# arclabs561/innr

Measured on NVIDIA B200. Metric: batch_knn_cosine_top10_queries_per_s, higher is better.
Workload: dtype f32

## Files before the change

innr_b200/csrc/scan_f32.cu:

```cuda
#include <algorithm>
#include <cmath>
#include <type_traits>

#include "common.cuh"
#include "kernels.cuh"
#include "pdx.cuh"

namespace innr {

namespace {

constexpr int SCAN_THREADS = 256;
constexpr int VPT = 4;
constexpr int TILE = SCAN_THREADS * VPT;
constexpr float NORM_EPS = 1e-9f;

struct PdxArgs {
  PdxView v;
  unsigned long long ld;
  unsigned n, d, ld4;
  unsigned n_tiles;
  unsigned index_base;
  const float* queries;
  int nq_valid;
  int k;
  uint64_t* partials;
  uint64_t* out_keys;
  uint64_t* group_partials;
  unsigned* tickets;
  float* scores_out;
  const float* norms_in;
  const uint32_t* mask;
  const uint32_t* perm;
  float threshold;
  float one;
  const unsigned* run_flag;
};

template <int MODE>
__device__ __forceinline__ void accumulate(float q, float v, float& acc) {
  if (MODE == PDX_L2 || MODE == PDX_L2_PRUNE || MODE == PDX_L2_PERM) {
    float diff = __fsub_rn(q, v);
    acc = __fadd_rn(acc, __fmul_rn(diff, diff));
  } else {
    acc = __fadd_rn(acc, __fmul_rn(q, v));
  }
}

template <int MODE>
__device__ __forceinline__ void accumulate2(uint64_t q2, uint64_t v2, uint64_t& acc2, uint64_t one2) {
  if (MODE == PDX_L2 || MODE == PDX_L2_PRUNE || MODE == PDX_L2_PERM) {
    const uint64_t diff = sub2_rn(q2, v2);
    acc2 = add2_unfusable(mul2_rn(diff, diff), acc2, one2);
  } else {
    acc2 = add2_unfusable(mul2_rn(q2, v2), acc2, one2);
  }
}

template <int MODE, int QB, int R, bool KNN, bool MASKED = false, int UX = 0>
// ... 943 lines not shown
  ++*launches;
  return cudaGetLastError();
}

cudaError_t launch_adaptive_epoch(const PdxView& v, const float* dev_query, size_t d0, size_t d1, float* dev_dist,
                                  const uint32_t* dev_mask_in, uint32_t* dev_mask_out, const float* dev_thr, uint32_t* dev_ev,
                                  unsigned* dev_pruned, int no_prune, cudaStream_t s, LaunchCounter* launches) {
  AdaptArgs a{};
  a.v = v;
  a.ld = v.ld;
  a.ld4 = (unsigned)std::min<size_t>(v.ld, (v.n + 3) / 4 * 4);
  a.query = dev_query;
  a.d0 = (unsigned)d0;
  a.d1 = (unsigned)d1;
  a.dist = dev_dist;
  a.mask_in = dev_mask_in;
  a.mask_out = dev_mask_out;
  a.thr = dev_thr;
  a.ev = dev_ev;
  a.pruned = dev_pruned;
  a.no_prune = no_prune;
  const unsigned span = (a.ld4 + 31u) / 32u * 32u;
  const unsigned grid = (span / VPT + SCAN_THREADS - 1) / SCAN_THREADS;
  adaptive_epoch_kernel<<<grid, SCAN_THREADS, (d1 - d0) * sizeof(float), s>>>(a);
  ++*launches;
  return cudaGetLastError();
}

cudaError_t launch_adaptive_event_keys(const uint32_t* dev_before, const uint32_t* dev_after, const uint32_t* dev_ev, size_t n,
                                       uint64_t* dev_keys, cudaStream_t s, LaunchCounter* launches) {
  adaptive_event_keys_kernel<<<(unsigned)((n + SCAN_THREADS - 1) / SCAN_THREADS), SCAN_THREADS, 0, s>>>(dev_before, dev_after,
                                                                                                     dev_ev, (unsigned)n, dev_keys);
  ++*launches;
  return cudaGetLastError();
}

cudaError_t launch_adaptive_revive(const uint64_t* dev_keys, size_t m, uint32_t* dev_mask, cudaStream_t s,
                                   LaunchCounter* launches) {
  if (m == 0) return cudaSuccess;
  adaptive_revive_kernel<<<(unsigned)((m + 255) / 256), 256, 0, s>>>(dev_keys, (unsigned)m, dev_mask);
  ++*launches;
  return cudaGetLastError();
}

cudaError_t launch_topk_from_distances(const float* dev_dist, size_t n, size_t k, uint64_t* dev_keys,
                                       Workspace& ws, cudaStream_t s, LaunchCounter* launches) {
  return launch_topk_from_scores(dev_dist, 0, n, 0, k, dev_keys, ws, s, launches, nullptr, nullptr, 1, 1);
}

namespace {

constexpr int SC_VPT = 16;
constexpr int SC_TILE = SCAN_THREADS * SC_VPT;
constexpr int SC_U = 8;
constexpr int RS_WARPS = 4;

struct ScreenArgs {
  PdxSketch sk;
  unsigned long long ld;
  unsigned n, d, ld16, n_tiles, index_base;
  int k;
  const float* query;
  const float* norms;
  float gamma, eta, nu;
  uint64_t* partials;
  uint64_t* group_partials;
  unsigned* tickets;
  uint64_t* tkeys;
  float* opt;
  float* pess;
  unsigned* ctl;
};

struct alignas(16) ScreenQuery {
  float qn_ref, qn_up;
  float qq_lo, qq_hi;
  float q128;
  float e1;
  float gq;
  float unscale;
  unsigned wmax[SCAN_THREADS / 32];
};

template <int MODE>
__device__ __forceinline__ void screen_bounds(float acc, float s, float r, float nv, const ScreenQuery& c,
                                              const ScreenArgs& a, float& lower, float& upper) {
  const float g = a.gamma;
  const float v_up = __fmul_ru(__fadd_ru(__fmul_ru(nv, 1.0f + 0x1p-23f), a.nu), __fadd_ru(1.0f, g));
  if (!(__fmul_ru(c.qn_up, v_up) <= 0x1p100f)) {
    lower = -INFINITY;
    upper = INFINITY;
    return;
  }
  const float m_lo = __fsub_rd(__fsub_rd(__fmul_rd(acc, c.unscale), c.q128), c.e1);
  const float m_hi = __fadd_ru(__fsub_ru(__fmul_ru(acc, c.unscale), c.q128), c.e1);
  const float qr = __fmul_ru(c.qn_up, r);
  const float x_lo = __fsub_rd(__fmul_rd(s, m_lo), qr);
  const float x_hi = __fadd_ru(__fmul_ru(s, m_hi), qr);
  if (MODE == PDX_L2) {
    const float n_lo = __fmul_rd(nv, 1.0f - 0x1p-23f);
    const float vv_lo = fmaxf(0.0f, __fmul_rd(__fsub_rd(__fmul_rd(n_lo, n_lo), a.eta), __fsub_rd(1.0f, g)));
    const float l_lo = fmaxf(0.0f, __fadd_rd(__fsub_rd(c.qq_lo, 2.0f * x_hi), vv_lo));
    const float l_hi = __fadd_ru(__fsub_ru(c.qq_hi, 2.0f * x_lo), __fmul_ru(v_up, v_up));
    lower = fmaxf(0.0f, __fsub_rd(__fmul_rd(l_lo, __fsub_rd(1.0f, g)), a.eta));
    upper = __fadd_ru(__fmul_ru(l_hi, __fadd_ru(1.0f, g)), a.eta);
    if (!(upper <= 3.0e38f)) { lower = -INFINITY; upper = INFINITY; }
    return;
  }
  const float e = __fmaf_ru(c.gq, v_up, a.eta);
  lower = __fsub_rd(x_lo, e);
  upper = __fadd_ru(x_hi, e);
  if (MODE == PDX_COSINE_FUSED) {
    if (!(nv > NORM_EPS)) {
      lower = upper = 0.0f;
      return;
    }
    const float p = __fmul_rn(c.qn_ref, nv);
    lower = __fdiv_rd(lower, p);
    upper = __fdiv_ru(upper, p);
  }
}

template <int MODE, int R>
__global__ void __launch_bounds__(SCAN_THREADS) pdx_screen_kernel(const ScreenArgs a) {
  extern __shared__ __align__(16) unsigned char smem_raw[];
  const unsigned d_pad = (a.d + 31u) / 32u * 32u;
  float* sq = reinterpret_cast<float*>(smem_raw);
  float* sqs = sq + d_pad;
  ScreenQuery* sc = reinterpret_cast<ScreenQuery*>(sqs + d_pad);
  uint64_t* smem_keys = reinterpret_cast<uint64_t*>(sc + 1);
  const int lane = threadIdx.x & 31;
  unsigned mb = 0;
  for (unsigned dd = threadIdx.x; dd < d_pad; dd += blockDim.x) {
    const float x = dd < a.d ? a.query[dd] : 0.0f;
    sq[dd] = x;
    mb = max(mb, __float_as_uint(x) & 0x7FFFFFFFu);
  }
  mb = __reduce_max_sync(FULL_MASK, mb);
  if (lane == 0) sc->wmax[threadIdx.x >> 5] = mb;
  __syncthreads();
#pragma unroll
  for (int w = 0; w < SCAN_THREADS / 32; ++w) mb = max(mb, sc->wmax[w]);
  if (!(mb >= 0x0D800000u && mb <= 0x71800000u)) {
    if (threadIdx.x == 0) a.ctl[1] = 1u;
    return;
  }
  const int p = 253 - (int)(mb >> 23);
  const float f1 = __uint_as_float((unsigned)(p / 2 + 127) << 23), f2 = __uint_as_float((unsigned)(p - p / 2 + 127) << 23);
  for (unsigned dd = threadIdx.x; dd < d_pad; dd += blockDim.x) sqs[dd] = __fmul_rn(__fmul_rn(sq[dd], f1), f2);
  __syncthreads();
  if (threadIdx.x == SCAN_THREADS - 1) {
    float ss = 0.0f, su = 0.0f, sl = 0.0f, qs = 0.0f, sa = 0.0f;
    for (unsigned dd = 0; dd < a.d; ++dd) {
      const float x = sq[dd];
      ss = __fadd_rn(ss, __fmul_rn(x, x));
      su = __fmaf_ru(x, x, su);
      sl = __fmaf_rd(x, x, sl);
      qs = __fadd_rn(qs, x);
      sa = __fadd_ru(sa, fabsf(x));
    }
    const float us = __uint_as_float((unsigned)(276 - p) << 23);
    sc->qn_ref = __fsqrt_rn(ss);
    sc->qn_up = __fsqrt_ru(su);
    sc->qq_lo = sl;
    sc->qq_hi = su;
    sc->q128 = 128.0f * qs;
    sc->e1 = __fadd_ru(__fmul_ru(a.gamma, __fmul_ru(383.0f, sa)), __fmul_ru(__uint_as_float(a.d), us));
    sc->gq = __fmul_ru(a.gamma, sc->qn_up);
    sc->unscale = us;
  }
  bool qn_visible = false;
  WarpList<R> lists[1];
  lists[0].init();
  uint64_t thr = KEY_SENTINEL;

  for (unsigned tile = blockIdx.x; tile < a.n_tiles; tile += gridDim.x) {
    const unsigned i0 = tile * SC_TILE + threadIdx.x * SC_VPT;
    const bool active = i0 < a.ld16;
    uint64_t acc[SC_VPT / 2];
#pragma unroll
    for (int j = 0; j < SC_VPT / 2; ++j) acc[j] = 0;
    auto step = [&](const uint4& w, float q) {
      const uint64_t q2 = pack2(q, q);
      const unsigned x[4] = {w.x, w.y, w.z, w.w};
#pragma unroll
      for (int t = 0; t < 4; ++t) {
        const float b0 = __uint_as_float(__byte_perm(x[t], 0u, 0x4440u)), b1 = __uint_as_float(__byte_perm(x[t], 0u, 0x4441u));
        const float b2 = __uint_as_float(__byte_perm(x[t], 0u, 0x4442u)), b3 = __uint_as_float(__byte_perm(x[t], 0u, 0x4443u));
        acc[2 * t] = fma2_rn(q2, pack2(b0, b1), acc[2 * t]);
        acc[2 * t + 1] = fma2_rn(q2, pack2(b2, b3), acc[2 * t + 1]);
      }
    };
    if (active) {
      const uint8_t* p = a.sk.codes + pdx_sketch_off(a.ld, 0, i0);
      const size_t next = pdx_sketch_off(a.ld, 1, 0);
      unsigned dd = 0;
      for (; dd + SC_U <= a.d; dd += SC_U) {
        uint4 w[SC_U];
#pragma unroll
        for (int u = 0; u < SC_U; ++u) w[u] = ldg_stream_u4(reinterpret_cast<const uint4*>(p + u * next));
        p += SC_U * next;
#pragma unroll
        for (int u = 0; u < SC_U; ++u) step(w[u], sqs[dd + u]);
      }
      for (; dd < a.d; ++dd, p += next) step(ldg_stream_u4(reinterpret_cast<const uint4*>(p)), sqs[dd]);
    }
    if (!qn_visible) {
      __syncthreads();
      qn_visible = true;
      const float qr = sc->qn_ref, qu = sc->qn_up;
      if (!(qu <= 0x1p100f) || (MODE == PDX_COSINE_FUSED && !(qr >= NORM_EPS))) {
        if (threadIdx.x == 0) a.ctl[1] = 1u;
        return;
      }
    }
#pragma unroll
    for (int h = 0; h < SC_VPT / 4; ++h) {
      const unsigned ih = i0 + 4 * h;
      float lo[4] = {0.0f, 0.0f, 0.0f, 0.0f}, up[4] = {0.0f, 0.0f, 0.0f, 0.0f};
      if (active) {
        const float4 s4 = *reinterpret_cast<const float4*>(a.sk.scale + ih);
        const float4 r4 = *reinterpret_cast<const float4*>(a.sk.resid + ih);
        const float4 n4 = *reinterpret_cast<const float4*>(a.norms + ih);
        const float s[4] = {s4.x, s4.y, s4.z, s4.w}, r[4] = {r4.x, r4.y, r4.z, r4.w}, nv[4] = {n4.x, n4.y, n4.z, n4.w};
        float x[4];
        unpack2(acc[2 * h], x[0], x[1]);
        unpack2(acc[2 * h + 1], x[2], x[3]);
#pragma unroll
        for (int j = 0; j < 4; ++j) screen_bounds<MODE>(x[j], s[j], r[j], nv[j], *sc, a, lo[j], up[j]);
        const float* ob = (MODE == PDX_L2) ? lo : up;
        *reinterpret_cast<float4*>(a.opt + ih) = make_float4(ob[0], ob[1], ob[2], ob[3]);
        if (a.pess) {
          const float* pb = (MODE == PDX_L2) ? up : lo;
          for (int j = 0; j < 4; ++j) a.pess[ih + j] = pb[j];
        }
      }
#pragma unroll
      for (int j = 0; j < 4; ++j) {
        const unsigned i = ih + j;
        const uint64_t key = (MODE == PDX_L2) ? make_key_asc(up[j], a.index_base + i) : make_key_desc(lo[j], a.index_base + i);
        lists[0].offer(key, active && i < a.n, thr, a.k, lane);
      }
    }
  }
  block_finish<R, 1>(lists, 1, a.k, smem_keys, a.partials, a.group_partials, a.tkeys, a.tickets);
}

__global__ void __launch_bounds__(SCAN_THREADS) screen_compact_kernel(const float* __restrict__ opt, unsigned n, int l2,
                                                                      const uint64_t* __restrict__ tkeys, int k,
                                                                      unsigned index_base, uint32_t* __restrict__ cand,
                                                                      unsigned* ctl) {
  if (ctl[1]) return;
  const uint64_t kth = tkeys[k - 1];
  float t;
  if (kth == KEY_SENTINEL) t = l2 ? INFINITY : -INFINITY;
  else t = __uint_as_float(order_bits_to_f32_bits(l2 ? (uint32_t)(kth >> 32) : ~(uint32_t)(kth >> 32)));
  const int lane = threadIdx.x & 31;
  const unsigned stride = gridDim.x * blockDim.x, n_round = (n + 31u) / 32u * 32u;
  for (unsigned i = blockIdx.x * blockDim.x + threadIdx.x; i < n_round; i += stride) {
    bool hit = false;
    if (i < n) {
      const float b = opt[i];
      hit = l2 ? !(b > t) : !(b < t);
    }
    const unsigned m = __ballot_sync(FULL_MASK, hit);
    if (!m) continue;
    unsigned base = 0;
    if (lane == 0) base = atomicAdd(&ctl[0], (unsigned)__popc(m));
    base = __shfl_sync(FULL_MASK, base, 0);
    const unsigned pos = base + __popc(m & ((1u << lane) - 1u));
    if (hit && pos < SCREEN_CAP) cand[pos] = index_base + i;
  }
}

template <int MODE>
__global__ void __launch_bounds__(RS_WARPS * 32) screen_rescore_kernel(const PdxView v, const float* __restrict__ query,
                                                                       const float* __restrict__ norms,
                                                                       const uint32_t* __restrict__ cand,
                                                                       unsigned* ctl, uint64_t* __restrict__ keys) {
  extern __shared__ __align__(16) unsigned char smem_raw[];
  const unsigned d = (unsigned)v.d, d_pad = (d + 3u) & ~3u;
  const int warp = threadIdx.x >> 5, lane = threadIdx.x & 31;
  float* sq = reinterpret_cast<float*>(smem_raw) + (size_t)2 * d_pad * warp;
  float* buf = sq + d_pad;
  const unsigned j = blockIdx.x * RS_WARPS + warp;
  const unsigned cnt = ctl[0], stop = ctl[1];
  if (j == 0 && lane == 0 && cnt > SCREEN_CAP) ctl[1] = 1u;
  if (stop || j >= min(cnt, (unsigned)SCREEN_CAP)) {
    if (lane == 0) keys[j] = KEY_SENTINEL;
    return;
  }
  for (unsigned dd = lane; dd < d; dd += 32) sq[dd] = query[dd];
  const unsigned gid = cand[j], i = gid - v.index_base;
  for (unsigned dd = lane; dd < d; dd += 32) buf[dd] = pdx_load1(v, (size_t)dd * v.ld + i);
  __syncwarp();
  if (lane != 0) return;
  float acc = 0.0f, qss = 0.0f;
  for (unsigned dd = 0; dd < d; ++dd) {
    const float q = sq[dd], x = buf[dd];
    accumulate<MODE == PDX_COSINE_FUSED ? PDX_DOT : MODE>(q, x, acc);
    if (MODE == PDX_COSINE_FUSED) qss = __fadd_rn(qss, __fmul_rn(q, q));
  }
  float sc = acc;
  if (MODE == PDX_COSINE_FUSED) {
    const float qn = __fsqrt_rn(qss), nrm = norms[i];
    sc = (!(qn < NORM_EPS) && nrm > NORM_EPS) ? __fdiv_rn(acc, __fmul_rn(qn, nrm)) : 0.0f;
  }
  keys[j] = MODE == PDX_L2 ? make_key_asc(sc, gid) : make_key_desc(sc, gid);
}

ScreenArgs screen_args(const PdxView& v, const float* dev_norms, const PdxSketch& sk, const float* dev_query, size_t k,
                       Workspace& ws) {
  ScreenArgs a{};
  a.sk = sk;
  a.ld = v.ld;
  a.n = (unsigned)v.n;
  a.d = (unsigned)v.d;
  a.ld16 = (unsigned)std::min<size_t>(v.ld, (v.n + 15) / 16 * 16);
  a.n_tiles = (unsigned)(((size_t)a.ld16 + SC_TILE - 1) / SC_TILE);
  a.index_base = v.index_base;
  a.k = (int)k;
  a.query = dev_query;
  a.norms = dev_norms;
  const double du = (double)(v.d + 2) * 0x1p-24;
  a.gamma = (float)(du / (1.0 - du)) * (1.0f + 0x1p-20f);
  a.eta = (float)((double)v.d * 0x1p-148) * (1.0f + 0x1p-20f) + 0x1p-149f;
  a.nu = (float)std::sqrt((double)v.d * 0x1p-149) * (1.0f + 0x1p-20f);
  a.partials = ws.partials;
  a.group_partials = ws.group_partials;
  a.tickets = ws.tickets;
  a.tkeys = ws.sc_keys + SCREEN_CAP;
  a.opt = ws.sc_bounds;
  a.ctl = ws.sc_ctl;
  return a;
}

template <int MODE, int R>
cudaError_t launch_screen(const ScreenArgs& a, int num_sms, cudaStream_t s) {
  auto kern = pdx_screen_kernel<MODE, R>;
  const size_t smem = (size_t)2 * ((a.d + 31u) / 32u * 32u) * sizeof(float) + sizeof(ScreenQuery) +
                      (size_t)(SCAN_THREADS / 32) * a.k * sizeof(uint64_t);
  static size_t smem_set_dev[16] = {};
  size_t& smem_set = smem_set_dev[current_device_slot()];
  if (smem > 48 * 1024 && smem > smem_set) {
    cudaError_t e = cudaFuncSetAttribute(kern, cudaFuncAttributeMaxDynamicSharedMemorySize, (int)smem);
    if (e != cudaSuccess) return e;
    smem_set = smem;
  }
  int occ = 0;
  cudaError_t e = cudaOccupancyMaxActiveBlocksPerMultiprocessor(&occ, kern, SCAN_THREADS, smem);
  if (e != cudaSuccess) return e;
  if (occ < 1) return cudaErrorInvalidConfiguration;
  kern<<<balanced_grid(a.n_tiles, (unsigned)occ * (unsigned)num_sms), SCAN_THREADS, smem, s>>>(a);
  return cudaGetLastError();
}

cudaError_t launch_screen_mode(int mode, const ScreenArgs& a, int num_sms, cudaStream_t s) {
  const bool big = a.k > 32;
  switch (mode) {
    case PDX_DOT: return big ? launch_screen<PDX_DOT, 4>(a, num_sms, s) : launch_screen<PDX_DOT, 1>(a, num_sms, s);
    case PDX_COSINE_FUSED:
      return big ? launch_screen<PDX_COSINE_FUSED, 4>(a, num_sms, s) : launch_screen<PDX_COSINE_FUSED, 1>(a, num_sms, s);
    case PDX_L2: return big ? launch_screen<PDX_L2, 4>(a, num_sms, s) : launch_screen<PDX_L2, 1>(a, num_sms, s);
  }
  return cudaErrorInvalidValue;
}

}

cudaError_t launch_pdx_knn_screened(const PdxView& v, int mode, const float* dev_norms, const PdxSketch& sk,
                                    const float* dev_query, size_t k, uint64_t* dev_keys, Workspace& ws, cudaStream_t s,
                                    LaunchCounter* launches) {
  if (!v.hi || !sk.codes || k == 0 || k > 128 || v.d == 0 || v.d > SCREEN_MAX_D || v.n < k || ws.sc_bounds_cap < v.ld)
    return cudaErrorInvalidValue;
  const ScreenArgs a = screen_args(v, dev_norms, sk, dev_query, k, ws);
  cudaError_t e = cudaMemsetAsync(ws.sc_ctl, 0, 2 * sizeof(unsigned), s);
  if (e != cudaSuccess) return e;
  if ((e = launch_screen_mode(mode, a, ws.num_sms, s)) != cudaSuccess) return e;
  screen_compact_kernel<<<(unsigned)std::min<size_t>((v.n + SCAN_THREADS - 1) / SCAN_THREADS, (size_t)ws.num_sms * 8), SCAN_THREADS, 0, s>>>(
      ws.sc_bounds, (unsigned)v.n, mode == PDX_L2, a.tkeys, (int)k, v.index_base, ws.sc_cand, ws.sc_ctl);
  const size_t rs_smem = (size_t)(2 * RS_WARPS) * ((v.d + 3) & ~(size_t)3) * sizeof(float);
#define INNR_RESCORE(MODE)                                                                                              \
  {                                                                                                                     \
    auto kern = screen_rescore_kernel<MODE>;                                                                            \
    if (rs_smem > 48 * 1024 && (e = cudaFuncSetAttribute(kern, cudaFuncAttributeMaxDynamicSharedMemorySize, (int)rs_smem)) != cudaSuccess) \
      return e;                                                                                                         \
    kern<<<(unsigned)(SCREEN_CAP / RS_WARPS), RS_WARPS * 32, rs_smem, s>>>(v, dev_query, dev_norms, ws.sc_cand, ws.sc_ctl, ws.sc_keys); \
  }
  if (mode == PDX_DOT) INNR_RESCORE(PDX_DOT)
  else if (mode == PDX_L2) INNR_RESCORE(PDX_L2)
  else INNR_RESCORE(PDX_COSINE_FUSED)
#undef INNR_RESCORE
  *launches += 3;
  if ((e = cudaGetLastError()) != cudaSuccess) return e;
  if ((e = launch_topk_from_scores(ws.sc_keys, 3, SCREEN_CAP, 0, k, dev_keys, ws, s, launches)) != cudaSuccess) return e;
  return launch_pdx_knn(v, mode, dev_query, 1, k, dev_keys, ws, s, launches, ws.sc_ctl + 1);
}

cudaError_t launch_pdx_screen_debug_bounds(const PdxView& v, int mode, const float* dev_norms, const PdxSketch& sk,
                                           const float* dev_query, float* host_lower, float* host_upper, Workspace& ws,
                                           cudaStream_t s, LaunchCounter* launches) {
  if (!v.hi || !sk.codes || v.n == 0 || v.d == 0 || v.d > SCREEN_MAX_D || 2 * v.ld > ws.sc_bounds_cap)
    return cudaErrorInvalidValue;
  ScreenArgs a = screen_args(v, dev_norms, sk, dev_query, 1, ws);
  a.pess = ws.sc_bounds + v.ld;
  cudaError_t e = cudaMemsetAsync(ws.sc_ctl, 0, 2 * sizeof(unsigned), s);
// ... 16 lines not shown
```

innr_b200/csrc/tc_common.cuh:

```cuda
#pragma once
#include <cuda.h>
#include <cuda_runtime.h>
#include <stdint.h>

namespace innr {
namespace tc {

__device__ __forceinline__ uint32_t smem_u32(const void* p) { return (uint32_t)__cvta_generic_to_shared(p); }

__device__ __forceinline__ void mbar_init(uint64_t* bar, uint32_t count) {
  asm volatile("mbarrier.init.shared::cta.b64 [%0], %1;" ::"r"(smem_u32(bar)), "r"(count) : "memory");
}
__device__ __forceinline__ void fence_barrier_init() {
  asm volatile("fence.mbarrier_init.release.cluster;" ::: "memory");
}
__device__ __forceinline__ void mbar_arrive_expect_tx(uint64_t* bar, uint32_t bytes) {
  asm volatile("mbarrier.arrive.expect_tx.shared::cta.b64 _, [%0], %1;" ::"r"(smem_u32(bar)), "r"(bytes) : "memory");
}
__device__ __forceinline__ void mbar_arrive(uint64_t* bar) {
  asm volatile("mbarrier.arrive.shared::cta.b64 _, [%0];" ::"r"(smem_u32(bar)) : "memory");
}
__device__ __forceinline__ bool mbar_try_wait(uint64_t* bar, uint32_t parity) {
  uint32_t ok;
  asm volatile(
      "{\n\t.reg .pred p;\n\t"
      "mbarrier.try_wait.parity.shared::cta.b64 p, [%1], %2;\n\t"
      "selp.u32 %0, 1, 0, p;\n\t}"
      : "=r"(ok)
      : "r"(smem_u32(bar)), "r"(parity)
      : "memory");
  return ok != 0;
}
__device__ __forceinline__ void mbar_wait(uint64_t* bar, uint32_t parity) {
  while (!mbar_try_wait(bar, parity)) {
  }
}

__device__ __forceinline__ void tma_prefetch_desc(const CUtensorMap* m) {
  asm volatile("prefetch.tensormap [%0];" ::"l"(m) : "memory");
}
__device__ __forceinline__ void tma_load_2d(void* smem_dst, const CUtensorMap* m, uint64_t* bar, int c0, int c1) {
  asm volatile(
      "cp.async.bulk.tensor.2d.shared::cluster.global.mbarrier::complete_tx::bytes [%0], [%1, {%3, %4}], [%2];"
      ::"r"(smem_u32(smem_dst)), "l"(m), "r"(smem_u32(bar)), "r"(c0), "r"(c1)
      : "memory");
}
__device__ __forceinline__ void fence_proxy_async_smem() {
  asm volatile("fence.proxy.async.shared::cta;" ::: "memory");
}

template <int NCOLS>
__device__ __forceinline__ void tmem_alloc(uint32_t* smem_dst) {
  asm volatile("tcgen05.alloc.cta_group::1.sync.aligned.shared::cta.b32 [%0], %1;" ::"r"(smem_u32(smem_dst)), "n"(NCOLS)
               : "memory");
  asm volatile("tcgen05.relinquish_alloc_permit.cta_group::1.sync.aligned;" ::: "memory");
}
template <int NCOLS>
__device__ __forceinline__ void tmem_dealloc(uint32_t taddr) {
  asm volatile("tcgen05.dealloc.cta_group::1.sync.aligned.b32 %0, %1;" ::"r"(taddr), "n"(NCOLS) : "memory");
}
__device__ __forceinline__ void tc_fence_before_sync() { asm volatile("tcgen05.fence::before_thread_sync;" ::: "memory"); }
__device__ __forceinline__ void tc_fence_after_sync() { asm volatile("tcgen05.fence::after_thread_sync;" ::: "memory"); }

__device__ __forceinline__ void umma_tf32(uint32_t d_tmem, uint64_t a_desc, uint64_t b_desc, uint32_t idesc,
                                          uint32_t accumulate) {
  asm volatile(
      "{\n\t.reg .pred p;\n\t"
      "setp.ne.b32 p, %4, 0;\n\t"
      "tcgen05.mma.cta_group::1.kind::tf32 [%0], %1, %2, %3, p;\n\t}"
      ::"r"(d_tmem), "l"(a_desc), "l"(b_desc), "r"(idesc), "r"(accumulate)
      : "memory");
}
__device__ __forceinline__ void umma_commit(uint64_t* bar) {
  asm volatile("tcgen05.commit.cta_group::1.mbarrier::arrive::one.shared::cluster.b64 [%0];" ::"r"(smem_u32(bar))
               : "memory");
}
__device__ __forceinline__ void tmem_ld_32x32b_x32(uint32_t taddr, uint32_t (&r)[32]) {
  asm volatile(
      "tcgen05.ld.sync.aligned.32x32b.x32.b32 "
      "{%0, %1, %2, %3, %4, %5, %6, %7, %8, %9, %10, %11, %12, %13, %14, %15, "
      "%16, %17, %18, %19, %20, %21, %22, %23, %24, %25, %26, %27, %28, %29, %30, %31}, [%32];"
      : "=r"(r[0]), "=r"(r[1]), "=r"(r[2]), "=r"(r[3]), "=r"(r[4]), "=r"(r[5]), "=r"(r[6]), "=r"(r[7]), "=r"(r[8]),
        "=r"(r[9]), "=r"(r[10]), "=r"(r[11]), "=r"(r[12]), "=r"(r[13]), "=r"(r[14]), "=r"(r[15]), "=r"(r[16]),
        "=r"(r[17]), "=r"(r[18]), "=r"(r[19]), "=r"(r[20]), "=r"(r[21]), "=r"(r[22]), "=r"(r[23]), "=r"(r[24]),
        "=r"(r[25]), "=r"(r[26]), "=r"(r[27]), "=r"(r[28]), "=r"(r[29]), "=r"(r[30]), "=r"(r[31])
      : "r"(taddr)
      : "memory");
}
__device__ __forceinline__ void tmem_st_32x32b_x32(uint32_t taddr, const uint32_t (&r)[32]) {
  asm volatile(
      "tcgen05.st.sync.aligned.32x32b.x32.b32 [%0], "
      "{%1, %2, %3, %4, %5, %6, %7, %8, %9, %10, %11, %12, %13, %14, %15, %16, "
      "%17, %18, %19, %20, %21, %22, %23, %24, %25, %26, %27, %28, %29, %30, %31, %32};"
      ::"r"(taddr), "r"(r[0]), "r"(r[1]), "r"(r[2]), "r"(r[3]), "r"(r[4]), "r"(r[5]), "r"(r[6]), "r"(r[7]), "r"(r[8]),
        "r"(r[9]), "r"(r[10]), "r"(r[11]), "r"(r[12]), "r"(r[13]), "r"(r[14]), "r"(r[15]), "r"(r[16]), "r"(r[17]),
        "r"(r[18]), "r"(r[19]), "r"(r[20]), "r"(r[21]), "r"(r[22]), "r"(r[23]), "r"(r[24]), "r"(r[25]), "r"(r[26]),
        "r"(r[27]), "r"(r[28]), "r"(r[29]), "r"(r[30]), "r"(r[31])
      : "memory");
// ... 107 lines not shown
```

innr_b200/csrc/u8.cu:

```cuda
#include <type_traits>

#include "common.cuh"
#include "kernels.cuh"
#include "pdx.cuh"
#include "tc_common.cuh"

namespace innr {

namespace {

constexpr int U8_THREADS = 256;
constexpr int U8_CTA = U8_THREADS + 32;
constexpr int U8_STAGE_CHUNKS = 4;
constexpr int U8_STAGES = 6;
constexpr int U8_ROW_BYTES = U8_THREADS * 16;
constexpr int U8_STAGE_BYTES = U8_STAGE_CHUNKS * U8_ROW_BYTES;

__device__ __forceinline__ float byte_to_f32_biased(unsigned word, int k, unsigned magic) {
  return __uint_as_float(__byte_perm(word, magic, 0x7440u | (unsigned)k));
}
__device__ __forceinline__ float byte_to_f32(unsigned word, int k, unsigned magic) {
  return __fsub_rn(byte_to_f32_biased(word, k, magic), 8388608.0f);
}

// ... 77 lines not shown
    float s = 0.0f;
#pragma unroll
    for (int e = 0; e < 16; ++e)
      if ((unsigned)e < d) s = __fadd_rn(s, __fmul_rn(sq[e], byte_to_f32(w[e >> 2], e & 3, magic)));
    return s;
  }
  float all[8];
#pragma unroll
  for (int j = 0; j < 8; ++j)
    all[j] = __fadd_rn(__fadd_rn(acc[j], acc[8 + j]), __fadd_rn(acc[16 + j], acc[24 + j]));
  float result = __fmul_rn(hsum8(all), unscale);
  const unsigned rs = (d / 32) * 32, remaining = d - rs, n8 = (remaining / 8) * 8;
  if (remaining == 0) return __fadd_rn(result, 0.0f);
  float rem[8];
#pragma unroll
  for (int j = 0; j < 8; ++j) rem[j] = 0.0f;
#pragma unroll
  for (int e = 0; e < 24; ++e)
    if ((unsigned)e < n8) rem[e & 7] = fmaf(sq[rs + e], byte_to_f32(w[e >> 2], e & 3, magic), rem[e & 7]);
  result = __fadd_rn(result, hsum8(rem));
#pragma unroll
  for (int e = 0; e < 31; ++e)
    if ((unsigned)e >= n8 && (unsigned)e < remaining)
      result = __fadd_rn(result, __fmul_rn(sq[rs + e], byte_to_f32(w[e >> 2], e & 3, magic)));
  return result;
}

struct U8Args {
  const uint4* data;
  unsigned long long ld;
  unsigned n, d, chunks, n_tiles, index_base;
  float alpha, offset;
  unsigned magic;
  int allow_scaled;
  const float* query;
  const float* query_b;
  int k, mode;
  uint64_t* partials;
  uint64_t* out_keys;
  uint64_t* group_partials;
  unsigned* tickets;
  float* scores_out;
};

int g_u8_allow_scaled = 1;

struct U8Shared {
  uint64_t full[U8_STAGES], empty[U8_STAGES];
};
constexpr int U8_PAIR_STAGES = 12;
struct U8PairShared {
  uint64_t full[U8_PAIR_STAGES], empty[U8_PAIR_STAGES];
};

__device__ __forceinline__ void bulk_load(void* smem_dst, const void* gsrc, unsigned bytes, uint64_t* bar) {
  asm volatile("cp.async.bulk.shared::cluster.global.mbarrier::complete_tx::bytes [%0], [%1], %2, [%3];"
               ::"r"(tc::smem_u32(smem_dst)), "l"(gsrc), "r"(bytes), "r"(tc::smem_u32(bar))
               : "memory");
}

template <int R, bool KNN>
__global__ void __launch_bounds__(U8_CTA, 2) u8_scan_kernel(const U8Args a) {
  extern __shared__ __align__(1024) unsigned char smem_raw[];
  unsigned char* ring = smem_raw;
  const unsigned d_pad = (a.d + 31) / 32 * 32 + 32;
  float* sq = reinterpret_cast<float*>(smem_raw + U8_STAGES * U8_STAGE_BYTES);
  float* s_misc = sq + d_pad;
  U8Shared* st = reinterpret_cast<U8Shared*>(s_misc + 4);
  uint64_t* smem_keys = reinterpret_cast<uint64_t*>(st + 1);
  const int lane = threadIdx.x & 31, warp = threadIdx.x >> 5;
  const bool producer = warp == U8_THREADS / 32;
  const unsigned main_elems = (a.d >= 16) ? (a.d / 32) * 32 : 0;
  bool q_ok = true;
  for (unsigned i = threadIdx.x; i < d_pad; i += blockDim.x) {
    const float v = i < a.d ? a.query[i] : 0.0f;
    sq[i] = v;
    if (i < main_elems) q_ok &= (v == 0.0f) || (fabsf(v) >= 0x1p-80f && fabsf(v) < 4.0f);
  }
  if (threadIdx.x == 0) {
    for (int sg = 0; sg < U8_STAGES; ++sg) {
      tc::mbar_init(&st->full[sg], 1);
      tc::mbar_init(&st->empty[sg], U8_THREADS / 32);
    }
    tc::fence_barrier_init();
  }
  const bool scaled = __syncthreads_and(q_ok) && a.allow_scaled;
  if (threadIdx.x == 32) {
    float s = 0.0f;
    for (unsigned i = 0; i < a.d; ++i) s = __fadd_rn(s, sq[i]);
    s_misc[0] = s;
  }
  __syncthreads();
  if (scaled) {
    for (unsigned i = threadIdx.x; i < main_elems; i += blockDim.x) sq[i] *= 0x1p126f;
    __syncthreads();
  }
  const float scale = __fdiv_rn(a.alpha, 255.0f);
  const float bias = __fmul_rn(a.offset, s_misc[0]);
  const unsigned stages_per_tile = (a.chunks + U8_STAGE_CHUNKS - 1) / U8_STAGE_CHUNKS;
  const unsigned main_chunks = (a.d >= 16) ? (a.d / 32) * 2 : 0;

  WarpList<R> lists[1];
  uint64_t thrs[1];
  lists[0].init();
  thrs[0] = KEY_SENTINEL;

  if (producer) {
    if (lane == 0) {
      unsigned slot = 0, phase = 1;
      for (unsigned tile = blockIdx.x; tile < a.n_tiles; tile += gridDim.x) {
        const unsigned long long col = (unsigned long long)tile * U8_THREADS;
        const unsigned long long left = a.ld - col;
        const unsigned row_bytes = (unsigned)(left < U8_THREADS ? left : U8_THREADS) * 16u;
        for (unsigned sgi = 0; sgi < stages_per_tile; ++sgi) {
          const unsigned c0 = sgi * U8_STAGE_CHUNKS;
          const unsigned rows = min((unsigned)U8_STAGE_CHUNKS, a.chunks - c0);
          while (!tc::mbar_try_wait(&st->empty[slot], phase)) __nanosleep(64);
          tc::mbar_arrive_expect_tx(&st->full[slot], rows * row_bytes);
          for (unsigned r = 0; r < rows; ++r)
            bulk_load(ring + slot * U8_STAGE_BYTES + r * U8_ROW_BYTES, a.data + (size_t)(c0 + r) * a.ld + col, row_bytes,
                      &st->full[slot]);
          if (++slot == U8_STAGES) { slot = 0; phase ^= 1; }
        }
      }
    }
  } else {
   auto consume = [&](auto scaled_tag) {
    constexpr bool SCALED = decltype(scaled_tag)::value;
    const unsigned full_stages = main_chunks / U8_STAGE_CHUNKS;
    unsigned slot = 0, phase = 0;
    const uint4* const ring_v = reinterpret_cast<const uint4*>(ring) + threadIdx.x;
    for (unsigned tile = blockIdx.x; tile < a.n_tiles; tile += gridDim.x) {
      const unsigned i = tile * U8_THREADS + threadIdx.x;
      const bool valid = i < a.n;
      float acc[32];
#pragma unroll
      for (int c = 0; c < 32; ++c) acc[c] = 0.0f;
      unsigned w[8] = {0, 0, 0, 0, 0, 0, 0, 0};
      unsigned sgi = 0;
      const float* qp = sq;
      for (; sgi < full_stages; ++sgi, qp += 16 * U8_STAGE_CHUNKS) {
        tc::mbar_wait(&st->full[slot], phase);
        const uint4* sv = ring_v + slot * (U8_STAGE_BYTES / 16);
        uint4 v[U8_STAGE_CHUNKS];
#pragma unroll
        for (int g = 0; g < U8_STAGE_CHUNKS; ++g) v[g] = sv[g * U8_THREADS];
        __syncwarp();
        if (lane == 0) tc::mbar_arrive(&st->empty[slot]);
        if (++slot == U8_STAGES) { slot = 0; phase ^= 1; }
#pragma unroll
        for (int g = 0; g < U8_STAGE_CHUNKS; ++g) fma16<SCALED>(v[g], qp + 16 * g, acc + 16 * (g & 1), a.magic);
      }
      for (; sgi < stages_per_tile; ++sgi) {
        const unsigned c0 = sgi * U8_STAGE_CHUNKS;
        tc::mbar_wait(&st->full[slot], phase);
        const uint4* sv = ring_v + slot * (U8_STAGE_BYTES / 16);
        uint4 v[U8_STAGE_CHUNKS];
#pragma unroll
        for (int g = 0; g < U8_STAGE_CHUNKS; ++g) v[g] = sv[g * U8_THREADS];
        __syncwarp();
        if (lane == 0) tc::mbar_arrive(&st->empty[slot]);
        if (++slot == U8_STAGES) { slot = 0; phase ^= 1; }
#pragma unroll
        for (int g = 0; g < U8_STAGE_CHUNKS; ++g) {
          const unsigned c = c0 + g;
          if (c < main_chunks) {
            fma16<SCALED>(v[g], sq + 16 * c, acc + 16 * (g & 1), a.magic);
          } else if (c < a.chunks) {
            if (c == main_chunks) { w[0] = v[g].x; w[1] = v[g].y; w[2] = v[g].z; w[3] = v[g].w; }
            else { w[4] = v[g].x; w[5] = v[g].y; w[6] = v[g].z; w[7] = v[g].w; }
          }
        }
      }
// ... 26 lines not shown
    const float va = i < a.d ? a.query[i] : 0.0f, vb = i < a.d ? a.query_b[i] : 0.0f;
    sqa[i] = va;
    sqb[i] = vb;
    if (i < main_elems)
      q_ok &= ((va == 0.0f) || (fabsf(va) >= 0x1p-80f && fabsf(va) < 4.0f)) &&
              ((vb == 0.0f) || (fabsf(vb) >= 0x1p-80f && fabsf(vb) < 4.0f));
  }
  if (threadIdx.x == 0) {
    for (int sg = 0; sg < U8_PAIR_STAGES; ++sg) {
      tc::mbar_init(&st->full[sg], 1);
      tc::mbar_init(&st->empty[sg], U8_THREADS / 32);
    }
    tc::fence_barrier_init();
  }
  const bool scaled = __syncthreads_and(q_ok) && a.allow_scaled;
  if (threadIdx.x == 32 || threadIdx.x == 64) {
    const float* qp = threadIdx.x == 64 ? sqb : sqa;
    float sum = 0.0f;
    for (unsigned i = 0; i < a.d; ++i) sum = __fadd_rn(sum, qp[i]);
    s_misc[threadIdx.x == 64 ? 1 : 0] = sum;
  }
  __syncthreads();
  if (scaled) {
    for (unsigned i = threadIdx.x; i < main_elems; i += blockDim.x) {
      sqa[i] *= 0x1p126f;
      sqb[i] *= 0x1p126f;
    }
    __syncthreads();
  }
  const float scale = __fdiv_rn(a.alpha, 255.0f);
  const float bias_a = __fmul_rn(a.offset, s_misc[0]), bias_b = __fmul_rn(a.offset, s_misc[1]);
  const unsigned stages_per_tile = (a.chunks + U8_STAGE_CHUNKS - 1) / U8_STAGE_CHUNKS;
  const unsigned main_chunks = (a.d >= 16) ? (a.d / 32) * 2 : 0;

  WarpList<R> lists[2];
  uint64_t thrs[2];
  lists[0].init();
  lists[1].init();
  thrs[0] = thrs[1] = KEY_SENTINEL;

  if (producer) {
    if (lane == 0) {
      unsigned slot = 0, phase = 1;
      for (unsigned tile = blockIdx.x; tile < a.n_tiles; tile += gridDim.x) {
        const unsigned long long col = (unsigned long long)tile * U8_THREADS;
        const unsigned long long left = a.ld - col;
        const unsigned row_bytes = (unsigned)(left < U8_THREADS ? left : U8_THREADS) * 16u;
        for (unsigned sgi = 0; sgi < stages_per_tile; ++sgi) {
          const unsigned c0 = sgi * U8_STAGE_CHUNKS;
          const unsigned rows = min((unsigned)U8_STAGE_CHUNKS, a.chunks - c0);
          while (!tc::mbar_try_wait(&st->empty[slot], phase)) __nanosleep(64);
          tc::mbar_arrive_expect_tx(&st->full[slot], rows * row_bytes);
          for (unsigned r = 0; r < rows; ++r)
            bulk_load(ring + slot * U8_STAGE_BYTES + r * U8_ROW_BYTES, a.data + (size_t)(c0 + r) * a.ld + col, row_bytes,
                      &st->full[slot]);
          if (++slot == U8_PAIR_STAGES) { slot = 0; phase ^= 1; }
        }
      }
    }
  } else {
    auto consume = [&](auto scaled_tag) {
      constexpr bool SCALED = decltype(scaled_tag)::value;
      unsigned slot = 0, phase = 0;
      const uint4* const ring_v = reinterpret_cast<const uint4*>(ring) + threadIdx.x;
      for (unsigned tile = blockIdx.x; tile < a.n_tiles; tile += gridDim.x) {
        const unsigned i = tile * U8_THREADS + threadIdx.x;
        const bool valid = i < a.n;
        float acc_a[32], acc_b[32];
#pragma unroll
        for (int c = 0; c < 32; ++c) acc_a[c] = acc_b[c] = 0.0f;
        unsigned w[8] = {0, 0, 0, 0, 0, 0, 0, 0};
        for (unsigned sgi = 0; sgi < stages_per_tile; ++sgi) {
          const unsigned c0 = sgi * U8_STAGE_CHUNKS;
          tc::mbar_wait(&st->full[slot], phase);
          const uint4* sv = ring_v + slot * (U8_STAGE_BYTES / 16);
          uint4 v[U8_STAGE_CHUNKS];
#pragma unroll
          for (int g = 0; g < U8_STAGE_CHUNKS; ++g) v[g] = sv[g * U8_THREADS];
          __syncwarp();
          if (lane == 0) tc::mbar_arrive(&st->empty[slot]);
          if (++slot == U8_PAIR_STAGES) { slot = 0; phase ^= 1; }
#pragma unroll
          for (int g = 0; g < U8_STAGE_CHUNKS; ++g) {
            const unsigned c = c0 + g;
            if (c < main_chunks) {
              fma16_pair<SCALED>(v[g], sqa + 16 * c, sqb + 16 * c, acc_a + 16 * (g & 1), acc_b + 16 * (g & 1), a.magic);
            } else if (c < a.chunks) {
              if (c == main_chunks) { w[0] = v[g].x; w[1] = v[g].y; w[2] = v[g].z; w[3] = v[g].w; }
              else { w[4] = v[g].x; w[5] = v[g].y; w[6] = v[g].z; w[7] = v[g].w; }
            }
          }
        }
        const float unscale = SCALED ? 0x1p23f : 1.0f;
        const float ma = mixed_dot_finish(acc_a, w, a.d, sqa, a.magic, unscale);
        const float mb = mixed_dot_finish(acc_b, w, a.d, sqb, a.magic, unscale);
        lists[0].offer(make_key_desc(__fadd_rn(__fmul_rn(scale, ma), bias_a), a.index_base + i), valid, thrs[0], a.k, lane);
        lists[1].offer(make_key_desc(__fadd_rn(__fmul_rn(scale, mb), bias_b), a.index_base + i), valid, thrs[1], a.k, lane);
      }
    };
    if (scaled) consume(std::true_type{}); else consume(std::false_type{});
  }
  block_finish<R, 2>(lists, 2, a.k, smem_keys, a.partials, a.group_partials, a.out_keys, a.tickets);
}

__global__ void u8_pack_kernel(const uint8_t* __restrict__ rows, unsigned n, unsigned d, uint4* __restrict__ codes,
                               size_t ld, unsigned chunks) {
  const size_t total = (size_t)chunks * ld;
// ... 214 lines not shown
```

Baseline: 777.3.

## Pipeline screen kernel sketch loads through TMA bulk-copy ring with producer warp

The sketch screen kernel now has a dedicated producer warp that streams the u8 code rows into a 5-stage shared-memory ring with cp.async.bulk and mbarriers, while 8 consumer warps compute from shared memory. A separate warp computes the query norms concurrently, and each CTA gets a contiguous balanced range of units instead of a strided tile loop. The goal is to hide global memory latency and free consumer registers, capped via __maxnreg__(80). The rescore kernel also batches its hi/lo loads to raise memory-level parallelism. The costs are mbarrier synchronisation overhead, more shared memory per block, and possible register spilling under the cap.

```diff
diff --git a/innr_b200/csrc/scan_f32.cu b/innr_b200/csrc/scan_f32.cu
--- a/innr_b200/csrc/scan_f32.cu
+++ b/innr_b200/csrc/scan_f32.cu
@@ -5,6 +5,7 @@
 #include "common.cuh"
 #include "kernels.cuh"
 #include "pdx.cuh"
+#include "tc_common.cuh"
 
 namespace innr {
 
@@ -1054,13 +1055,18 @@
 
 constexpr int SC_VPT = 16;
 constexpr int SC_TILE = SCAN_THREADS * SC_VPT;
-constexpr int SC_U = 8;
+constexpr int SC_STAGE_DIMS = 4;
+constexpr int SC_STAGE_BYTES = SC_STAGE_DIMS * SC_TILE;
+constexpr int SC_STAGES = 5;
+constexpr int SC_CTA = SCAN_THREADS + 64;
+constexpr int SC_PRODUCER = SCAN_THREADS / 32, SC_QUERY = SC_PRODUCER + 1;
 constexpr int RS_WARPS = 4;
+constexpr int RS_BATCH = 8;
 
 struct ScreenArgs {
   PdxSketch sk;
   unsigned long long ld;
-  unsigned n, d, ld16, n_tiles, index_base;
+  unsigned n, d, ld16, index_base;
   int k;
   const float* query;
   const float* norms;
@@ -1081,7 +1087,12 @@
   float e1;
   float gq;
   float unscale;
-  unsigned wmax[SCAN_THREADS / 32];
+  unsigned wmax[SC_CTA / 32];
+};
+
+struct ScreenRing {
+  uint64_t full[SC_STAGES], empty[SC_STAGES], q_ready;
+  unsigned refused;
 };
 
 template <int MODE>
@@ -1124,14 +1135,16 @@
 }
 
 template <int MODE, int R>
-__global__ void __launch_bounds__(SCAN_THREADS) pdx_screen_kernel(const ScreenArgs a) {
+__global__ void __maxnreg__(80) pdx_screen_kernel(const ScreenArgs a) {
   extern __shared__ __align__(16) unsigned char smem_raw[];
+  unsigned char* ring = smem_raw;
   const unsigned d_pad = (a.d + 31u) / 32u * 32u;
-  float* sq = reinterpret_cast<float*>(smem_raw);
+  float* sq = reinterpret_cast<float*>(smem_raw + SC_STAGES * SC_STAGE_BYTES);
   float* sqs = sq + d_pad;
   ScreenQuery* sc = reinterpret_cast<ScreenQuery*>(sqs + d_pad);
-  uint64_t* smem_keys = reinterpret_cast<uint64_t*>(sc + 1);
-  const int lane = threadIdx.x & 31;
+  ScreenRing* st = reinterpret_cast<ScreenRing*>(sc + 1);
+  uint64_t* smem_keys = reinterpret_cast<uint64_t*>(st + 1);
+  const int lane = threadIdx.x & 31, warp = threadIdx.x >> 5;
   unsigned mb = 0;
   for (unsigned dd = threadIdx.x; dd < d_pad; dd += blockDim.x) {
     const float x = dd < a.d ? a.query[dd] : 0.0f;
@@ -1139,10 +1152,19 @@
     mb = max(mb, __float_as_uint(x) & 0x7FFFFFFFu);
   }
   mb = __reduce_max_sync(FULL_MASK, mb);
-  if (lane == 0) sc->wmax[threadIdx.x >> 5] = mb;
+  if (lane == 0) sc->wmax[warp] = mb;
+  if (threadIdx.x == 0) {
+    for (int sg = 0; sg < SC_STAGES; ++sg) {
+      tc::mbar_init(&st->full[sg], 1);
+      tc::mbar_init(&st->empty[sg], SCAN_THREADS / 32);
+    }
+    tc::mbar_init(&st->q_ready, 1);
+    st->refused = 0u;
+    tc::fence_barrier_init();
+  }
   __syncthreads();
 #pragma unroll
-  for (int w = 0; w < SCAN_THREADS / 32; ++w) mb = max(mb, sc->wmax[w]);
+  for (int w = 0; w < SC_CTA / 32; ++w) mb = max(mb, sc->wmax[w]);
   if (!(mb >= 0x0D800000u && mb <= 0x71800000u)) {
     if (threadIdx.x == 0) a.ctl[1] = 1u;
     return;
@@ -1151,99 +1173,158 @@
   const float f1 = __uint_as_float((unsigned)(p / 2 + 127) << 23), f2 = __uint_as_float((unsigned)(p - p / 2 + 127) << 23);
   for (unsigned dd = threadIdx.x; dd < d_pad; dd += blockDim.x) sqs[dd] = __fmul_rn(__fmul_rn(sq[dd], f1), f2);
   __syncthreads();
-  if (threadIdx.x == SCAN_THREADS - 1) {
-    float ss = 0.0f, su = 0.0f, sl = 0.0f, qs = 0.0f, sa = 0.0f;
-    for (unsigned dd = 0; dd < a.d; ++dd) {
-      const float x = sq[dd];
-      ss = __fadd_rn(ss, __fmul_rn(x, x));
-      su = __fmaf_ru(x, x, su);
-      sl = __fmaf_rd(x, x, sl);
-      qs = __fadd_rn(qs, x);
-      sa = __fadd_ru(sa, fabsf(x));
-    }
-    const float us = __uint_as_float((unsigned)(276 - p) << 23);
-    sc->qn_ref = __fsqrt_rn(ss);
-    sc->qn_up = __fsqrt_ru(su);
-    sc->qq_lo = sl;
-    sc->qq_hi = su;
-    sc->q128 = 128.0f * qs;
-    sc->e1 = __fadd_ru(__fmul_ru(a.gamma, __fmul_ru(383.0f, sa)), __fmul_ru(__uint_as_float(a.d), us));
-    sc->gq = __fmul_ru(a.gamma, sc->qn_up);
-    sc->unscale = us;
-  }
-  bool qn_visible = false;
+
+  const unsigned units = a.ld16 / 16u;
+  const unsigned u_begin = (unsigned)((unsigned long long)units * blockIdx.x / gridDim.x);
+  const unsigned u_len = (unsigned)((unsigned long long)units * (blockIdx.x + 1) / gridDim.x) - u_begin;
+  const unsigned n_sub = (u_len + SCAN_THREADS - 1) / SCAN_THREADS;
+  auto sub = [&](unsigned s) { return u_begin + (unsigned)((unsigned long long)u_len * s / n_sub); };
+  const unsigned n_stages = (a.d + SC_STAGE_DIMS - 1) / SC_STAGE_DIMS;
+  auto refused = [&]() {
+    tc::mbar_wait(&st->q_ready, 0);
+    return *reinterpret_cast<volatile unsigned*>(&st->refused) != 0u;
+  };
+
   WarpList<R> lists[1];
   lists[0].init();
   uint64_t thr = KEY_SENTINEL;
 
-  for (unsigned tile = blockIdx.x; tile < a.n_tiles; tile += gridDim.x) {
-    const unsigned i0 = tile * SC_TILE + threadIdx.x * SC_VPT;
-    const bool active = i0 < a.ld16;
-    uint64_t acc[SC_VPT / 2];
-#pragma unroll
-    for (int j = 0; j < SC_VPT / 2; ++j) acc[j] = 0;
-    auto step = [&](const uint4& w, float q) {
-      const uint64_t q2 = pack2(q, q);
-      const unsigned x[4] = {w.x, w.y, w.z, w.w};
-#pragma unroll
-      for (int t = 0; t < 4; ++t) {
-        const float b0 = __uint_as_float(__byte_perm(x[t], 0u, 0x4440u)), b1 = __uint_as_float(__byte_perm(x[t], 0u, 0x4441u));
-        const float b2 = __uint_as_float(__byte_perm(x[t], 0u, 0x4442u)), b3 = __uint_as_float(__byte_perm(x[t], 0u, 0x4443u));
-        acc[2 * t] = fma2_rn(q2, pack2(b0, b1), acc[2 * t]);
-        acc[2 * t + 1] = fma2_rn(q2, pack2(b2, b3), acc[2 * t + 1]);
-      }
-    };
-    if (active) {
-      const uint8_t* p = a.sk.codes + pdx_sketch_off(a.ld, 0, i0);
-      const size_t next = pdx_sketch_off(a.ld, 1, 0);
-      unsigned dd = 0;
-      for (; dd + SC_U <= a.d; dd += SC_U) {
-        uint4 w[SC_U];
-#pragma unroll
-        for (int u = 0; u < SC_U; ++u) w[u] = ldg_stream_u4(reinterpret_cast<const uint4*>(p + u * next));
-        p += SC_U * next;
-#pragma unroll
-        for (int u = 0; u < SC_U; ++u) step(w[u], sqs[dd + u]);
-      }
-      for (; dd < a.d; ++dd, p += next) step(ldg_stream_u4(reinterpret_cast<const uint4*>(p)), sqs[dd]);
-    }
-    if (!qn_visible) {
-      __syncthreads();
-      qn_visible = true;
-      const float qr = sc->qn_ref, qu = sc->qn_up;
-      if (!(qu <= 0x1p100f) || (MODE == PDX_COSINE_FUSED && !(qr >= NORM_EPS))) {
-        if (threadIdx.x == 0) a.ctl[1] = 1u;
-        return;
-      }
-    }
-#pragma unroll
-    for (int h = 0; h < SC_VPT / 4; ++h) {
-      const unsigned ih = i0 + 4 * h;
-      float lo[4] = {0.0f, 0.0f, 0.0f, 0.0f}, up[4] = {0.0f, 0.0f, 0.0f, 0.0f};
-      if (active) {
-        const float4 s4 = *reinterpret_cast<const float4*>(a.sk.scale + ih);
-        const float4 r4 = *reinterpret_cast<const float4*>(a.sk.resid + ih);
-        const float4 n4 = *reinterpret_cast<const float4*>(a.norms + ih);
-        const float s[4] = {s4.x, s4.y, s4.z, s4.w}, r[4] = {r4.x, r4.y, r4.z, r4.w}, nv[4] = {n4.x, n4.y, n4.z, n4.w};
-        float x[4];
-        unpack2(acc[2 * h], x[0], x[1]);
-        unpack2(acc[2 * h + 1], x[2], x[3]);
-#pragma unroll
-        for (int j = 0; j < 4; ++j) screen_bounds<MODE>(x[j], s[j], r[j], nv[j], *sc, a, lo[j], up[j]);
-        const float* ob = (MODE == PDX_L2) ? lo : up;
-        *reinterpret_cast<float4*>(a.opt + ih) = make_float4(ob[0], ob[1], ob[2], ob[3]);
-        if (a.pess) {
-          const float* pb = (MODE == PDX_L2) ? up : lo;
-          for (int j = 0; j < 4; ++j) a.pess[ih + j] = pb[j];
+  if (warp == SC_PRODUCER) {
+    if (lane == 0) {
+      unsigned issued = 0;
+      bool stop = false;
+      for (unsigned s = 0; s < n_sub && !stop; ++s) {
+        const unsigned c0 = sub(s), bytes = (sub(s + 1) - c0) * 16u;
+        const uint8_t* src = a.sk.codes + pdx_sketch_off(a.ld, 0, (size_t)c0 * 16u);
+        for (unsigned g = 0; g < n_stages; ++g, ++issued) {
+          const unsigned slot = issued % SC_STAGES, phase = ((issued / SC_STAGES) & 1u) ^ 1u;
+          while (!tc::mbar_try_wait(&st->empty[slot], phase)) {
+            if (s > 0 && *reinterpret_cast<volatile unsigned*>(&st->refused)) { stop = true; break; }
+            __nanosleep(64);
+          }
+          if (stop) break;
+          const unsigned rows = min((unsigned)SC_STAGE_DIMS, a.d - g * SC_STAGE_DIMS);
+          tc::mbar_arrive_expect_tx(&st->full[slot], rows * bytes);
+          for (unsigned r = 0; r < rows; ++r)
+            tc::bulk_load(ring + slot * SC_STAGE_BYTES + r * SC_TILE, src + pdx_sketch_off(a.ld, g * SC_STAGE_DIMS + r, 0),
+                          bytes, &st->full[slot]);
         }
       }
-#pragma unroll
-      for (int j = 0; j < 4; ++j) {
-        const unsigned i = ih + j;
-        const uint64_t key = (MODE == PDX_L2) ? make_key_asc(up[j], a.index_base + i) : make_key_desc(lo[j], a.index_base + i);
-        lists[0].offer(key, active && i < a.n, thr, a.k, lane);
-      }
-    }
+      for (unsigned j = issued > SC_STAGES ? issued - SC_STAGES : 0u; j < issued; ++j)
+        tc::mbar_wait(&st->full[j % SC_STAGES], (j / SC_STAGES) & 1u);
+    }
+    __syncwarp();
+    if (refused()) return;
+  } else if (warp == SC_QUERY) {
+    bool no = false;
+    if (lane == 0) {
+      float ss = 0.0f, su = 0.0f, sl = 0.0f, qs = 0.0f, sa = 0.0f;
+      for (unsigned dd = 0; dd < a.d; ++dd) {
+        const float x = sq[dd];
+        ss = __fadd_rn(ss, __fmul_rn(x, x));
+        su = __fmaf_ru(x, x, su);
+        sl = __fmaf_rd(x, x, sl);
+        qs = __fadd_rn(qs, x);
+        sa = __fadd_ru(sa, fabsf(x));
+      }
+      const float us = __uint_as_float((unsigned)(276 - p) << 23);
+      const float qr = __fsqrt_rn(ss), qu = __fsqrt_ru(su);
+      sc->qn_ref = qr;
+      sc->qn_up = qu;
+      sc->qq_lo = sl;
+      sc->qq_hi = su;
+      sc->q128 = 128.0f * qs;
+      sc->e1 = __fadd_ru(__fmul_ru(a.gamma, __fmul_ru(383.0f, sa)), __fmul_ru(__uint_as_float(a.d), us));
+      sc->gq = __fmul_ru(a.gamma, qu);
+      sc->unscale = us;
+      no = !(qu <= 0x1p100f) || (MODE == PDX_COSINE_FUSED && !(qr >= NORM_EPS));
+      if (no) {
+        a.ctl[1] = 1u;
+        st->refused = 1u;
+      }
+      tc::mbar_arrive(&st->q_ready);
+    }
+    if (__shfl_sync(FULL_MASK, (unsigned)no, 0)) return;
+  } else {
+    unsigned slot = 0, phase = 0;
+    const uint4* const ring_v = reinterpret_cast<const uint4*>(ring) + threadIdx.x;
+    const float4* const sqs4 = reinterpret_cast<const float4*>(sqs);
+    const unsigned full_stages = a.d / SC_STAGE_DIMS, tail = a.d % SC_STAGE_DIMS;
+    for (unsigned s = 0; s < n_sub; ++s) {
+      const unsigned c0 = sub(s);
+      const bool active = threadIdx.x < sub(s + 1) - c0;
+      const unsigned i0 = (c0 + threadIdx.x) * SC_VPT;
+      uint64_t acc[SC_VPT / 2];
+#pragma unroll
+      for (int j = 0; j < SC_VPT / 2; ++j) acc[j] = 0;
+      auto step = [&](const uint4& w, float q) {
+        const uint64_t q2 = pack2(q, q);
+        const unsigned x[4] = {w.x, w.y, w.z, w.w};
+#pragma unroll
+        for (int t = 0; t < 4; ++t) {
+          const float b0 = __uint_as_float(__byte_perm(x[t], 0u, 0x4440u)), b1 = __uint_as_float(__byte_perm(x[t], 0u, 0x4441u));
+          const float b2 = __uint_as_float(__byte_perm(x[t], 0u, 0x4442u)), b3 = __uint_as_float(__byte_perm(x[t], 0u, 0x4443u));
+          acc[2 * t] = fma2_rn(q2, pack2(b0, b1), acc[2 * t]);
+          acc[2 * t + 1] = fma2_rn(q2, pack2(b2, b3), acc[2 * t + 1]);
+        }
+      };
+      auto take = [&](uint4 (&w)[SC_STAGE_DIMS]) {
+        tc::mbar_wait(&st->full[slot], phase);
+        const uint4* sv = ring_v + slot * (SC_STAGE_BYTES / 16);
+#pragma unroll
+        for (int r = 0; r < SC_STAGE_DIMS; ++r) w[r] = sv[r * (SC_TILE / 16)];
+        __syncwarp();
+        if (lane == 0) tc::mbar_arrive(&st->empty[slot]);
+        if (++slot == SC_STAGES) { slot = 0; phase ^= 1u; }
+      };
+      for (unsigned g = 0; g < full_stages; ++g) {
+        uint4 w[SC_STAGE_DIMS];
+        take(w);
+        const float4 q = sqs4[g];
+        step(w[0], q.x);
+        step(w[1], q.y);
+        step(w[2], q.z);
+        step(w[3], q.w);
+      }
+      if (tail) {
+        uint4 w[SC_STAGE_DIMS];
+        take(w);
+        const float4 q = sqs4[full_stages];
+        step(w[0], q.x);
+        if (tail > 1) step(w[1], q.y);
+        if (tail > 2) step(w[2], q.z);
+      }
+      if (s == 0 && refused()) return;
+#pragma unroll
+      for (int h = 0; h < SC_VPT / 4; ++h) {
+        const unsigned ih = i0 + 4 * h;
+        float lo[4] = {0.0f, 0.0f, 0.0f, 0.0f}, up[4] = {0.0f, 0.0f, 0.0f, 0.0f};
+        if (active) {
+          const float4 s4 = *reinterpret_cast<const float4*>(a.sk.scale + ih);
+          const float4 r4 = *reinterpret_cast<const float4*>(a.sk.resid + ih);
+          const float4 n4 = *reinterpret_cast<const float4*>(a.norms + ih);
+          const float sv[4] = {s4.x, s4.y, s4.z, s4.w}, r[4] = {r4.x, r4.y, r4.z, r4.w}, nv[4] = {n4.x, n4.y, n4.z, n4.w};
+          float x[4];
+          unpack2(acc[2 * h], x[0], x[1]);
+          unpack2(acc[2 * h + 1], x[2], x[3]);
+#pragma unroll
+          for (int j = 0; j < 4; ++j) screen_bounds<MODE>(x[j], sv[j], r[j], nv[j], *sc, a, lo[j], up[j]);
+          const float* ob = (MODE == PDX_L2) ? lo : up;
+          *reinterpret_cast<float4*>(a.opt + ih) = make_float4(ob[0], ob[1], ob[2], ob[3]);
+          if (a.pess) {
+            const float* pb = (MODE == PDX_L2) ? up : lo;
+            for (int j = 0; j < 4; ++j) a.pess[ih + j] = pb[j];
+          }
+        }
+#pragma unroll
+        for (int j = 0; j < 4; ++j) {
+          const unsigned i = ih + j;
+          const uint64_t key = (MODE == PDX_L2) ? make_key_asc(up[j], a.index_base + i) : make_key_desc(lo[j], a.index_base + i);
+          lists[0].offer(key, active && i < a.n, thr, a.k, lane);
+        }
+      }
+    }
+    if (n_sub == 0 && refused()) return;
   }
   block_finish<R, 1>(lists, 1, a.k, smem_keys, a.partials, a.group_partials, a.tkeys, a.tickets);
 }
@@ -1292,9 +1373,30 @@
     if (lane == 0) keys[j] = KEY_SENTINEL;
     return;
   }
-  for (unsigned dd = lane; dd < d; dd += 32) sq[dd] = query[dd];
   const unsigned gid = cand[j], i = gid - v.index_base;
-  for (unsigned dd = lane; dd < d; dd += 32) buf[dd] = pdx_load1(v, (size_t)dd * v.ld + i);
+  const uint16_t* hi = v.hi + i;
+  const uint16_t* lo = v.lo + i;
+  for (unsigned d0 = 0; d0 < d; d0 += 32u * RS_BATCH) {
+    float qv[RS_BATCH];
+    uint16_t h[RS_BATCH], l[RS_BATCH];
+#pragma unroll
+    for (int u = 0; u < RS_BATCH; ++u) {
+      const unsigned dd = d0 + 32u * u + lane;
+      if (dd < d) {
+        qv[u] = query[dd];
+        h[u] = __ldg(hi + (size_t)dd * v.ld);
+        l[u] = __ldg(lo + (size_t)dd * v.ld);
+      }
+    }
+#pragma unroll
+    for (int u = 0; u < RS_BATCH; ++u) {
+      const unsigned dd = d0 + 32u * u + lane;
+      if (dd < d) {
+        sq[dd] = qv[u];
+        buf[dd] = __uint_as_float(((uint32_t)h[u] << 16) | (uint32_t)l[u]);
+      }
+    }
+  }
   __syncwarp();
   if (lane != 0) return;
   float acc = 0.0f, qss = 0.0f;
@@ -1319,7 +1421,6 @@
   a.n = (unsigned)v.n;
   a.d = (unsigned)v.d;
   a.ld16 = (unsigned)std::min<size_t>(v.ld, (v.n + 15) / 16 * 16);
-  a.n_tiles = (unsigned)(((size_t)a.ld16 + SC_TILE - 1) / SC_TILE);
   a.index_base = v.index_base;
   a.k = (int)k;
   a.query = dev_query;
@@ -1340,20 +1441,20 @@
 template <int MODE, int R>
 cudaError_t launch_screen(const ScreenArgs& a, int num_sms, cudaStream_t s) {
   auto kern = pdx_screen_kernel<MODE, R>;
-  const size_t smem = (size_t)2 * ((a.d + 31u) / 32u * 32u) * sizeof(float) + sizeof(ScreenQuery) +
-                      (size_t)(SCAN_THREADS / 32) * a.k * sizeof(uint64_t);
+  const size_t smem = (size_t)SC_STAGES * SC_STAGE_BYTES + (size_t)2 * ((a.d + 31u) / 32u * 32u) * sizeof(float) +
+                      sizeof(ScreenQuery) + sizeof(ScreenRing) + (size_t)(SC_CTA / 32) * a.k * sizeof(uint64_t);
   static size_t smem_set_dev[16] = {};
   size_t& smem_set = smem_set_dev[current_device_slot()];
-  if (smem > 48 * 1024 && smem > smem_set) {
+  if (smem > smem_set) {
     cudaError_t e = cudaFuncSetAttribute(kern, cudaFuncAttributeMaxDynamicSharedMemorySize, (int)smem);
     if (e != cudaSuccess) return e;
     smem_set = smem;
   }
   int occ = 0;
-  cudaError_t e = cudaOccupancyMaxActiveBlocksPerMultiprocessor(&occ, kern, SCAN_THREADS, smem);
+  cudaError_t e = cudaOccupancyMaxActiveBlocksPerMultiprocessor(&occ, kern, SC_CTA, smem);
   if (e != cudaSuccess) return e;
   if (occ < 1) return cudaErrorInvalidConfiguration;
-  kern<<<balanced_grid(a.n_tiles, (unsigned)occ * (unsigned)num_sms), SCAN_THREADS, smem, s>>>(a);
+  kern<<<(unsigned)occ * (unsigned)num_sms, SC_CTA, smem, s>>>(a);
   return cudaGetLastError();
 }
 
diff --git a/innr_b200/csrc/tc_common.cuh b/innr_b200/csrc/tc_common.cuh
--- a/innr_b200/csrc/tc_common.cuh
+++ b/innr_b200/csrc/tc_common.cuh
@@ -44,6 +44,11 @@
       "cp.async.bulk.tensor.2d.shared::cluster.global.mbarrier::complete_tx::bytes [%0], [%1, {%3, %4}], [%2];"
       ::"r"(smem_u32(smem_dst)), "l"(m), "r"(smem_u32(bar)), "r"(c0), "r"(c1)
       : "memory");
+}
+__device__ __forceinline__ void bulk_load(void* smem_dst, const void* gsrc, unsigned bytes, uint64_t* bar) {
+  asm volatile("cp.async.bulk.shared::cluster.global.mbarrier::complete_tx::bytes [%0], [%1], %2, [%3];"
+               ::"r"(smem_u32(smem_dst)), "l"(gsrc), "r"(bytes), "r"(smem_u32(bar))
+               : "memory");
 }
 __device__ __forceinline__ void fence_proxy_async_smem() {
   asm volatile("fence.proxy.async.shared::cta;" ::: "memory");
diff --git a/innr_b200/csrc/u8.cu b/innr_b200/csrc/u8.cu
--- a/innr_b200/csrc/u8.cu
+++ b/innr_b200/csrc/u8.cu
@@ -153,12 +153,6 @@
 struct U8PairShared {
   uint64_t full[U8_PAIR_STAGES], empty[U8_PAIR_STAGES];
 };
-
-__device__ __forceinline__ void bulk_load(void* smem_dst, const void* gsrc, unsigned bytes, uint64_t* bar) {
-  asm volatile("cp.async.bulk.shared::cluster.global.mbarrier::complete_tx::bytes [%0], [%1], %2, [%3];"
-               ::"r"(tc::smem_u32(smem_dst)), "l"(gsrc), "r"(bytes), "r"(tc::smem_u32(bar))
-               : "memory");
-}
 
 template <int R, bool KNN>
 __global__ void __launch_bounds__(U8_CTA, 2) u8_scan_kernel(const U8Args a) {
@@ -219,7 +213,7 @@
           while (!tc::mbar_try_wait(&st->empty[slot], phase)) __nanosleep(64);
           tc::mbar_arrive_expect_tx(&st->full[slot], rows * row_bytes);
           for (unsigned r = 0; r < rows; ++r)
-            bulk_load(ring + slot * U8_STAGE_BYTES + r * U8_ROW_BYTES, a.data + (size_t)(c0 + r) * a.ld + col, row_bytes,
+            tc::bulk_load(ring + slot * U8_STAGE_BYTES + r * U8_ROW_BYTES, a.data + (size_t)(c0 + r) * a.ld + col, row_bytes,
                       &st->full[slot]);
           if (++slot == U8_STAGES) { slot = 0; phase ^= 1; }
         }
@@ -352,7 +346,7 @@
           while (!tc::mbar_try_wait(&st->empty[slot], phase)) __nanosleep(64);
           tc::mbar_arrive_expect_tx(&st->full[slot], rows * row_bytes);
           for (unsigned r = 0; r < rows; ++r)
-            bulk_load(ring + slot * U8_STAGE_BYTES + r * U8_ROW_BYTES, a.data + (size_t)(c0 + r) * a.ld + col, row_bytes,
+            tc::bulk_load(ring + slot * U8_STAGE_BYTES + r * U8_ROW_BYTES, a.data + (size_t)(c0 + r) * a.ld + col, row_bytes,
                       &st->full[slot]);
           if (++slot == U8_PAIR_STAGES) { slot = 0; phase ^= 1; }
         }
```

Result: no change. 774.6, median of 6 (-0.3%).
